# youngers2006/Dreamer

Hardware: AMD Instinct MI355X
Metric: imagined latent-steps/sec (B×H) at 64×64 CarRacing, 1/2/4/8 MI355X (higher is better)
Workload: dtype f32; 1 GPU; Dreamer.train_Agent() with AC_epochs=1 (replay sample + warm start S/2 + H-step imagination + actor-critic update), B=256/GPU S=64 H=15 64x64x3, precision=fp32 (north-star batch per GPU); global_batch=256, seq_len=64, horizon=15, parallelism=dp1, precision=fp32

## Files before the change

### dreamer_amd/csrc/conv_split.hip

```cpp
#include "conv.h"

#include <algorithm>
#include <climits>
#include <type_traits>

namespace {
typedef unsigned short u16;
typedef __bf16 bf16x8 __attribute__((ext_vector_type(8)));
typedef unsigned u32x4 __attribute__((ext_vector_type(4)));
typedef unsigned u32x2 __attribute__((ext_vector_type(2)));

__device__ __forceinline__ f32x4 mfma_b16(u32x4 a, u32x4 b, f32x4 c) {
  return __builtin_amdgcn_mfma_f32_16x16x32_bf16(__builtin_bit_cast(bf16x8, a), __builtin_bit_cast(bf16x8, b), c, 0, 0,
                                                  0);
}
__device__ __forceinline__ unsigned b16bits(__bf16 v) { return (unsigned)__builtin_bit_cast(u16, v); }
__device__ __forceinline__ void split3(float x, unsigned& h, unsigned& m, unsigned& l) {
  const __bf16 bh = (__bf16)x;
  const float r1 = x - (float)bh;
  const __bf16 bm = (__bf16)r1;
  const float r2 = r1 - (float)bm;
  h = b16bits(bh);
  m = b16bits(bm);
  l = b16bits((__bf16)r2);
}
__device__ __forceinline__ int swz(int row) { return (0x1320 >> (((row >> 2) & 3) * 4)) & 3; }
__device__ __forceinline__ u32x2 pack_bf16x4(f32x4 v) {
  typedef __bf16 bf16x4_t __attribute__((ext_vector_type(4)));
  const bf16x4_t b = {(__bf16)v[0], (__bf16)v[1], (__bf16)v[2], (__bf16)v[3]};
  return __builtin_bit_cast(u32x2, b);
}
__device__ __forceinline__ unsigned pack_bf16x2(float x0, float x1) { return b16bits((__bf16)x0) | (b16bits((__bf16)x1) << 16); }
}

template <int CIN>
__device__ __forceinline__ void conv_chunk(int c, int& tap, int& ci0, int& kc) {
  constexpr int CPT = CIN / 32;
  const int cc = c >> 4, t = c & 15;
  const int g = t >> 2, j = t & 3;
  const int ky = (g >> 1) + 2 * (j >> 1), kx = (g & 1) + 2 * (j & 1);
  tap = ky * 4 + kx;
  ci0 = 32 * cc;
  kc = tap * CPT + cc;
}

template <int BM, int BN, int CIN, bool OUT_NCHW, int PIPE, int EPI = CONV_EPI_FWD, int NT3 = 3, bool IO16 = (NT3 == 1)>
__global__ __launch_bounds__(BM * 2) void k_conv_split3(int n_frames, int ih, int iw, int cout,
                                                         const float* __restrict__ in, const u16* __restrict__ wr,
                                                         const float* __restrict__ bias, float* __restrict__ out,
                                                         float* __restrict__ pre) {
  static_assert(NT3 == 3 || (NT3 == 1 && (EPI == CONV_EPI_FWD || !IO16)), "conv_split3 terms");
  static_assert(!IO16 || NT3 == 1, "bf16 storage is the one-term form's");
  const u16* __restrict__ in16 = reinterpret_cast<const u16*>(in);
  u16* __restrict__ out16 = reinterpret_cast<u16*>(out);
  constexpr int NT = BM * 2;
  constexpr int K = CIN * 16;
  constexpr int NCH = K / 32;
  constexpr int WTN = BN / 2, FM = 4, FN = WTN / 16;
  constexpr int APT = BM * 8 / NT;
  constexpr int BU = NT3 * BN * 4;
  constexpr int BPT = (BU + NT - 1) / NT;
  static_assert(CIN % 32 == 0 && APT == 4 && FN >= 1, "conv_split3 tile");
  __shared__ __attribute__((aligned(16))) u32x4 As[2][NT3][BM][4];
  __shared__ __attribute__((aligned(16))) u32x4 Bs[2][NT3][BN][4];

  const int oh = ih / 2, ow = iw / 2, hw = oh * ow;
  const long long M = (long long)n_frames * hw;
  const int tiles_n = cout / BN;
  const long long tiles = ((M + BM - 1) / BM) * tiles_n;
  const int lt = dr_xcd_tile(blockIdx.x, (int)tiles);
  if (lt < 0) return;
  const long long m0 = (long long)(lt / tiles_n) * BM;
  const int n0 = (lt % tiles_n) * BN;
  const int tid = threadIdx.x, wave = tid >> 6, lane = tid & 63, r = lane & 15, q = lane >> 4;
  const int quad = tid & 7, prow = tid >> 3;

  int pb[APT];
  unsigned vm[APT];
#pragma unroll
  for (int i = 0; i < APT; ++i) {
    const long long m = m0 + prow + (NT / 8) * i;
    const int mm = (int)(m < M ? m : 0);
    const int f = mm / hw, p = mm - f * hw, oy = p / ow, ox = p - oy * ow;
    const int y0 = 2 * oy - 1, x0 = 2 * ox - 1;
    pb[i] = ((f * ih + y0) * iw + x0) * CIN;
    unsigned v = 0u;
#pragma unroll
    for (int t = 0; t < 4; ++t) {
      v |= (y0 + t >= 0 && y0 + t < ih) ? (1u << t) : 0u;
      v |= (x0 + t >= 0 && x0 + t < iw) ? (16u << t) : 0u;
    }
    vm[i] = m < M ? v : 0u;
  }

  f32x4 ra0[APT], ra1[APT];
  u32x2 rh0[APT], rh1[APT];
  u32x4 rb0[BPT], rb1[BPT];
  unsigned ok0 = 0, ok1 = 0;
  auto load = [&](int c, auto slot) __attribute__((always_inline)) {
    f32x4* ra = decltype(slot)::value == 0 ? ra0 : ra1;
    u32x2* rh = decltype(slot)::value == 0 ? rh0 : rh1;
    unsigned& okm = decltype(slot)::value == 0 ? ok0 : ok1;
    u32x4* rb = decltype(slot)::value == 0 ? rb0 : rb1;
    int tap, ci0, kc;
    conv_chunk<CIN>(c, tap, ci0, kc);
    const int ky = tap >> 2, kx = tap & 3;
    const int toff = (ky * iw + kx) * CIN + ci0 + 4 * quad;
    unsigned om = 0u;
#pragma unroll
    for (int i = 0; i < APT; ++i) {
      const bool ok = (vm[i] >> ky) & (vm[i] >> (4 + kx)) & 1u;
      if constexpr (IO16) rh[i] = *reinterpret_cast<const u32x2*>(in16 + (ok ? pb[i] + toff : 0));
      else ra[i] = *reinterpret_cast<const f32x4*>(in + (ok ? pb[i] + toff : 0));
      om |= ok ? (1u << i) : 0u;
    }
    okm = om;
#pragma unroll
    for (int j = 0; j < BPT; ++j) {
      const int e = tid + NT * j;
      if (BU % NT == 0 || e < BU) {
        const int pl = e / (BN * 4), rem = e - pl * BN * 4, row = rem >> 2, u = rem & 3;
        rb[j] = *reinterpret_cast<const u32x4*>(wr + (((long long)kc * 3 + pl) * cout + n0 + row) * 32 + 8 * u);
      }
    }
  };
  auto store = [&](auto slot, int buf) __attribute__((always_inline)) {
    const f32x4* ra = decltype(slot)::value == 0 ? ra0 : ra1;
    const u32x2* rh = decltype(slot)::value == 0 ? rh0 : rh1;
    const u32x4* rb = decltype(slot)::value == 0 ? rb0 : rb1;
    const unsigned okm = decltype(slot)::value == 0 ? ok0 : ok1;
#pragma unroll
    for (int i = 0; i < APT; ++i) {
      const int row = prow + (NT / 8) * i;
      const int unit = (quad >> 1) ^ swz(row), half = quad & 1;
      if constexpr (IO16) {
        reinterpret_cast<u32x2*>(&As[buf][0][row][unit])[half] = (okm >> i) & 1u ? rh[i] : (u32x2){0u, 0u};
      } else if constexpr (NT3 == 1) {
        const f32x4 v = (okm >> i) & 1u ? ra[i] : (f32x4){0.f, 0.f, 0.f, 0.f};
        reinterpret_cast<u32x2*>(&As[buf][0][row][unit])[half] = pack_bf16x4(v);
      } else {
        const f32x4 v = (okm >> i) & 1u ? ra[i] : (f32x4){0.f, 0.f, 0.f, 0.f};
        unsigned h0, m0_, l0, h1, m1, l1;
        split3_pair(v[0], v[1], h0, m0_, l0);
        split3_pair(v[2], v[3], h1, m1, l1);
        reinterpret_cast<u32x2*>(&As[buf][0][row][unit])[half] = (u32x2){h0, h1};
        reinterpret_cast<u32x2*>(&As[buf][1][row][unit])[half] = (u32x2){m0_, m1};
        reinterpret_cast<u32x2*>(&As[buf][2][row][unit])[half] = (u32x2){l0, l1};
      }
    }
#pragma unroll
    for (int j = 0; j < BPT; ++j) {
      const int e = tid + NT * j;
      if (BU % NT == 0 || e < BU) {
        const int pl = e / (BN * 4), rem = e - pl * BN * 4, row = rem >> 2, u = rem & 3;
        Bs[buf][pl][row][u ^ swz(row)] = rb[j];
      }
    }
  };

  const int wm0 = (wave >> 1) * 64, wn0 = (wave & 1) * WTN;
  const int fu = q ^ swz(r);
  f32x4 acc[FM][FN];
#pragma unroll
  for (int i = 0; i < FM; ++i)
#pragma unroll
    for (int j = 0; j < FN; ++j) acc[i][j] = (f32x4){0.f, 0.f, 0.f, 0.f};

  using S0 = std::integral_constant<int, 0>;
  using S1 = std::integral_constant<int, 1>;
  load(0, S0{});
  load(1, S1{});
  store(S0{}, 0);
  __syncthreads();
  auto step = [&](int c, auto slot) __attribute__((always_inline)) {
    constexpr int SL = decltype(slot)::value;
    using Next = std::integral_constant<int, 1 - SL>;
    const int buf = c & 1;
    load(min(c + PIPE, NCH - 1), slot);
    u32x4 a[NT3][FM], b[NT3][FN];
#pragma unroll
    for (int pl = 0; pl < NT3; ++pl) {
#pragma unroll
      for (int i = 0; i < FM; ++i) a[pl][i] = As[buf][pl][wm0 + 16 * i + r][fu];
#pragma unroll
      for (int j = 0; j < FN; ++j) b[pl][j] = Bs[buf][pl][wn0 + 16 * j + r][fu];
    }
#define DR_S3(PA, PB)                                                                                   \
  _Pragma("unroll") for (int i = 0; i < FM; ++i) _Pragma("unroll") for (int j = 0; j < FN; ++j) acc[i][j] = \
      OUT_NCHW ? mfma_b16(a[PA][i], b[PB][j], acc[i][j]) : mfma_b16(b[PB][j], a[PA][i], acc[i][j]);
    if constexpr (NT3 == 3) {
      DR_S3(2, 0)
      DR_S3(1, 1)
      DR_S3(0, 2)
      DR_S3(1, 0)
      DR_S3(0, 1)
    }
    DR_S3(0, 0)
#undef DR_S3
    if (c + 1 < NCH) store(Next{}, buf ^ 1);
    dr_lds_barrier();
  };
  static_assert(PIPE == 2 && NCH % 2 == 0, "conv_split3 ring");
  for (int c = 0; c < NCH; c += 2) {
    step(c, S0{});
    step(c + 1, S1{});
  }

#pragma unroll
  for (int i = 0; i < FM; ++i)
#pragma unroll
    for (int j = 0; j < FN; ++j) {
      if (OUT_NCHW) {
        const long long m = m0 + wm0 + 16 * i + 4 * q;
        const int co = n0 + wn0 + 16 * j + r;
        if (m >= M) continue;
        const float bv = bias[co];
        f32x4 v = acc[i][j] + bv;
        if constexpr (IO16) {
#pragma unroll
          for (int e = 0; e < 4; ++e) v[e] = dr_silu_fast(v[e]);
          const long long f = m / hw;
          *reinterpret_cast<u32x2*>(out16 + (f * cout + co) * hw + (m - f * hw)) = pack_bf16x4(v);
          continue;
        }
        if (pre) {
#pragma unroll
          for (int e = 0; e < 4; ++e) pre[(m + e) * cout + co] = v[e];
        }
#pragma unroll
        for (int e = 0; e < 4; ++e) v[e] = dr_silu_fast(v[e]);
        const long long f = m / hw;
        *reinterpret_cast<f32x4*>(out + (f * cout + co) * hw + (m - f * hw)) = v;
      } else {
        const long long m = m0 + wm0 + 16 * i + r;
        const int co = n0 + wn0 + 16 * j + 4 * q;
        if (m >= M) continue;
        f32x4 v;
        if (EPI == CONV_EPI_DSILU) {
          const f32x4 pv = *reinterpret_cast<const f32x4*>(pre + m * cout + co);
#pragma unroll
          for (int e = 0; e < 4; ++e) v[e] = acc[i][j][e] * dr_dsilu_fast(pv[e]);
        } else {
          const f32x4 bv = *reinterpret_cast<const f32x4*>(bias + co);
#pragma unroll
          for (int e = 0; e < 4; ++e) v[e] = acc[i][j][e] + bv[e];
          if (pre) *reinterpret_cast<f32x4*>(pre + m * cout + co) = v;
#pragma unroll
          for (int e = 0; e < 4; ++e) v[e] = dr_silu_fast(v[e]);
        }
        if constexpr (IO16) {
          *reinterpret_cast<u32x2*>(out16 + m * cout + co) = pack_bf16x4(v);
          continue;
        }
        *reinterpret_cast<f32x4*>(out + m * cout + co) = v;
      }
    }
}

__device__ __forceinline__ void conv_repack_split3_elem(int i, int cout, int cin, const float* __restrict__ w,
                                                        u16* __restrict__ wr) {
  const int co = i / (16 * cin), k = i - co * 16 * cin;
  const int tap = k / cin, ci = k - tap * cin;
  unsigned h, m, l;
  split3(w[((long long)co * cin + ci) * 16 + tap], h, m, l);
  const long long base = ((long long)(k >> 5) * 3 * cout + co) * 32 + (k & 31), plane = (long long)cout * 32;
  wr[base] = (u16)h;
  wr[base + plane] = (u16)m;
  wr[base + 2 * plane] = (u16)l;
}
__global__ void k_conv_repack_split3(int cout, int cin, const float* __restrict__ w, u16* __restrict__ wr) {
  const int i = blockIdx.x * blockDim.x + threadIdx.x;
  if (i >= cout * 16 * cin) return;
  conv_repack_split3_elem(i, cout, cin, w, wr);
}

int op_conv_repack_split3(int cout, int cin, const float* w, void* wr, hipStream_t s) {
  const int total = cout * 16 * cin;
  hipLaunchKernelGGL(k_conv_repack_split3, dim3((total + 255) / 256), dim3(256), 0, s, cout, cin, w, (u16*)wr);
  return dr_check_launch("conv_repack_split3");
}

#define E12_R2 8
#define E12_R1 (2 * E12_R2 + 2)
#define E12_RI (2 * E12_R1 + 2)
#define E12_PS (E12_R1 * 32 + 1)
#define E12_LWI 66
static constexpr size_t e12_lds_bytes(int terms = 3) {
  return (size_t)terms * 4 * E12_PS * 16 + (size_t)E12_RI * E12_LWI * 8;
}

#define DR_E12S1_WAVES 4
#define DR_E12S1_OCC 2
template <int NW, int NTM = 3, bool O16 = (NTM == 1)>
__global__ __launch_bounds__(64 * NW, NTM == 1 ? DR_E12S1_OCC : 1) void k_enc12_split3(int n, int nb, dr_frames src, const u16* __restrict__ wr1,
                                                          const float* __restrict__ b1, const u16* __restrict__ wr2,
                                                          const float* __restrict__ b2, float* __restrict__ out,
                                                          float* __restrict__ pre0, float* __restrict__ a0,
                                                          float* __restrict__ pre1) {
  static_assert((NW == 4 || NW == 8) && (NTM == 1 || NTM == 3) && (!O16 || NTM == 1), "enc12 waves / terms");
  constexpr int NTH = 64 * NW, TAPS = NW == 8 ? 8 : 16;
  constexpr int R2 = E12_R2, R1 = E12_R1, RI = E12_RI, PS = E12_PS, LWI = E12_LWI;
  constexpr int OW1 = 32, OW2 = 16, W = 64, H = 64, C1 = 32, C2 = 64;
  extern __shared__ __attribute__((aligned(16))) u32x4 e12_smem[];
  u32x4* c1o = e12_smem;
  uint2* xin = reinterpret_cast<uint2*>(e12_smem + NTM * 4 * PS);
  u16* xs = reinterpret_cast<u16*>(xin);
  u16* c1h = reinterpret_cast<u16*>(c1o);
  const int tid = threadIdx.x, wave = tid >> 6, lane = tid & 63, r = lane & 15, q = lane >> 4;
  const int ntiles = 2 * n;
  int tile = blockIdx.x;
  if (tile >= ntiles) return;

  for (int i = tid; i < RI * LWI; i += NTH) xin[i] = make_uint2(0u, 0u);
  constexpr int W4 = W / 4, PERC = RI * W4, MAXI = (3 * PERC + NTH - 1) / NTH;
  const unsigned hw = (unsigned)(H * W);
  const float centre = src.raw255 ? 127.5f : 0.0f, scale = src.raw255 ? 1.0f / 255.0f : 1.0f;
  unsigned uv[MAXI];
  auto in_load = [&](int tl) __attribute__((always_inline)) {
    const int f = tl >> 1, iy0 = 2 * (2 * (tl & 1) * R2 - 1) - 1;
    const int b = f % nb, t = f / nb + src.t0;
    const unsigned char* fr8 = src.ring + ((src.starts[b] + t) % src.ring_cap) * 3 * (long long)hw;
#pragma unroll
    for (int k = 0; k < MAXI; ++k) {
      const int i = tid + NTH * k;
      const int c = i / PERC, rem = i - c * PERC, rr = rem / W4, x4 = rem - rr * W4;
      const int y = iy0 + rr;
      const bool ok = i < 3 * PERC && y >= 0 && y < H;
      uv[k] = *reinterpret_cast<const unsigned*>(fr8 + (ok ? (unsigned)c * hw + (unsigned)(y * W + 4 * x4) : 0u));
    }
  };
  auto in_store = [&](int tl) __attribute__((always_inline)) {
    const int iy0 = 2 * (2 * (tl & 1) * R2 - 1) - 1;
#pragma unroll
    for (int k = 0; k < MAXI; ++k) {
      const int i = tid + NTH * k;
      if (i >= 3 * PERC) continue;
      const int c = i / PERC, rem = i - c * PERC, rr = rem / W4, x4 = rem - rr * W4;
      const int y = iy0 + rr;
      const bool ok = y >= 0 && y < H;
#pragma unroll
      for (int e = 0; e < 4; ++e)
        xs[(rr * LWI + 4 * x4 + e + 1) * 4 + c] =
            ok ? b16bits((__bf16)((float)((uv[k] >> (8 * e)) & 255u) - centre)) : (u16)0;
    }
  };
  in_load(tile);
  __syncthreads();
  in_store(tile);
  __syncthreads();

  const int w4 = wave & 3, kh = wave >> 2, ph = w4 & 1, ch = w4 >> 1;
  const u16* wbase = wr2 + ((long long)(32 * ch + r)) * 32 + 8 * q;
  auto wld = [&](u32x4 (&wf)[NTM][2], int tap) __attribute__((always_inline)) {
#pragma unroll
    for (int pl = 0; pl < NTM; ++pl)
#pragma unroll
      for (int jj = 0; jj < 2; ++jj)
        wf[pl][jj] = *reinterpret_cast<const u32x4*>(wbase + ((long long)(tap * 3 + pl) * C2 + 16 * jj) * 32);
  };

  for (;;) {
    const int f = tile >> 1, y2_0 = (tile & 1) * R2, y1_0 = 2 * y2_0 - 1;
    const int next = tile + (int)gridDim.x;
    u32x4 wa1[NTM][2][2];
#pragma unroll
    for (int pl = 0; pl < NTM; ++pl)
#pragma unroll
      for (int s = 0; s < 2; ++s)
#pragma unroll
        for (int j = 0; j < 2; ++j)
          wa1[pl][s][j] = *reinterpret_cast<const u32x4*>(wr1 + ((long long)pl * C1 + 16 * j + r) * 64 + 32 * s + 8 * q);
    float bb1[2][4];
#pragma unroll
    for (int j = 0; j < 2; ++j)
#pragma unroll
      for (int e = 0; e < 4; ++e) bb1[j][e] = b1[16 * j + 4 * q + e];
    u32x4 wfa[NTM][2], wfb[NTM][2];
    wld(wfa, TAPS * kh);
    constexpr int F1 = R1 * OW1 / 16;
    for (int i = wave; i < F1; i += NW) {
      const int p0 = 16 * i, yl = p0 / OW1, x1 = p0 - yl * OW1 + r, p = p0 + r;
      const int y1 = y1_0 + yl;
      uint2 hv[2], mv[2], lv[2];
      if (y1 < 0 || y1 >= H / 2) {
#pragma unroll
        for (int j = 0; j < 2; ++j) hv[j] = mv[j] = lv[j] = make_uint2(0u, 0u);
      } else {
        f32x4 acc[2] = {(f32x4){0.f, 0.f, 0.f, 0.f}, (f32x4){0.f, 0.f, 0.f, 0.f}};
#pragma unroll
        for (int s = 0; s < 2; ++s) {
          const int t0 = 8 * s + 2 * q, ky = t0 >> 2, kx = t0 & 3;
          const u32x4 pb = *reinterpret_cast<const u32x4*>(&xin[(2 * yl + ky) * LWI + 2 * x1 + kx]);
#pragma unroll
          for (int j = 0; j < 2; ++j) {
#pragma unroll
            for (int pl = NTM - 1; pl >= 0; --pl) acc[j] = mfma_b16(wa1[pl][s][j], pb, acc[j]);
          }
        }
        const bool own = !O16 && pre0 && yl >= 1 && yl <= 2 * R2;
        const long long o1 = (((long long)f * (H / 2) + y1) * OW1 + x1) * C1;
#pragma unroll
        for (int j = 0; j < 2; ++j) {
          float v[4], pv[4];
#pragma unroll
          for (int e = 0; e < 4; ++e) {
            pv[e] = acc[j][e] * scale + bb1[j][e];
            v[e] = dr_silu_fast(pv[e]);
          }
          if (own) {
            *reinterpret_cast<f32x4*>(pre0 + o1 + 16 * j + 4 * q) = (f32x4){pv[0], pv[1], pv[2], pv[3]};
            *reinterpret_cast<f32x4*>(a0 + o1 + 16 * j + 4 * q) = (f32x4){v[0], v[1], v[2], v[3]};
          }
          if constexpr (NTM == 1) {
            const u32x2 pk = pack_bf16x4((f32x4){v[0], v[1], v[2], v[3]});
            hv[j] = make_uint2(pk[0], pk[1]);
          } else {
            split3_pair(v[0], v[1], hv[j].x, mv[j].x, lv[j].x);
            split3_pair(v[2], v[3], hv[j].y, mv[j].y, lv[j].y);
          }
        }
      }
#pragma unroll
      for (int j = 0; j < 2; ++j) {
        const int c8 = 2 * j + (q >> 1);
        const int o = (c8 * PS + p) * 8 + (q & 1) * 4;
        *reinterpret_cast<uint2*>(c1h + o) = hv[j];
        if constexpr (NTM == 3) {
          *reinterpret_cast<uint2*>(c1h + 4 * PS * 8 + o) = mv[j];
          *reinterpret_cast<uint2*>(c1h + 2 * 4 * PS * 8 + o) = lv[j];
        }
      }
    }
    __syncthreads();
    if (next < ntiles) in_load(next);

    f32x4 acc[4][2];
#pragma unroll
    for (int i = 0; i < 4; ++i)
#pragma unroll
      for (int jj = 0; jj < 2; ++jj) acc[i][jj] = (f32x4){0.f, 0.f, 0.f, 0.f};
    auto tap_step = [&](int tap, u32x4 (&wf)[NTM][2], u32x4 (&wn)[NTM][2]) __attribute__((always_inline)) {
      wld(wn, tap + 1 < TAPS * (kh + 1) ? tap + 1 : tap);
      const int ky = tap >> 2, kx = tap & 3;
      const int x1 = 2 * r - 1 + kx;
      const bool xok = x1 >= 0 && x1 < OW1;
      u32x4 pf[NTM][4];
#pragma unroll
      for (int i = 0; i < 4; ++i) {
        const int yl = 2 * (4 * ph + i) + ky;
        const int u = q * PS + yl * OW1 + (xok ? x1 : 0);
#pragma unroll
        for (int pl = 0; pl < NTM; ++pl) {
          const u32x4 v = c1o[pl * 4 * PS + u];
          pf[pl][i] = xok ? v : (u32x4){0u, 0u, 0u, 0u};
        }
      }
#define E12_S3(PW, PA)                       \
  _Pragma("unroll") for (int i = 0; i < 4; ++i) _Pragma("unroll") for (int jj = 0; jj < 2; ++jj) acc[i][jj] = \
      mfma_b16(wf[PW][jj], pf[PA][i], acc[i][jj]);
      if constexpr (NTM == 3) {
        E12_S3(2, 0)
        E12_S3(1, 1)
        E12_S3(0, 2)
        E12_S3(1, 0)
        E12_S3(0, 1)
      }
      E12_S3(0, 0)
#undef E12_S3
    };
#pragma unroll 1
    for (int tap = TAPS * kh; tap < TAPS * (kh + 1); ++tap) {
      tap_step(tap, wfa, wfb);
#pragma unroll
      for (int pl = 0; pl < NTM; ++pl)
#pragma unroll
        for (int jj = 0; jj < 2; ++jj) wfa[pl][jj] = wfb[pl][jj];
    }
    if (NW == 8) {
      f32x4* red = reinterpret_cast<f32x4*>(e12_smem);
      __syncthreads();
      if (kh == 1) {
#pragma unroll
        for (int i = 0; i < 4; ++i)
#pragma unroll
          for (int jj = 0; jj < 2; ++jj) red[(w4 * 8 + i * 2 + jj) * 64 + lane] = acc[i][jj];
      }
      __syncthreads();
      if (kh == 0) {
#pragma unroll
        for (int i = 0; i < 4; ++i)
#pragma unroll
          for (int jj = 0; jj < 2; ++jj) acc[i][jj] += red[(w4 * 8 + i * 2 + jj) * 64 + lane];
      }
    }
#pragma unroll
    for (int i = 0; i < 4; ++i) {
      if (kh) break;
      float* o = out + (((long long)f * OW2 + y2_0 + 4 * ph + i) * OW2 + r) * C2;
#pragma unroll
      for (int jj = 0; jj < 2; ++jj) {
        const int co = 32 * ch + 16 * jj + 4 * q;
        const f32x4 bv = *reinterpret_cast<const f32x4*>(b2 + co);
        f32x4 v;
        const f32x4 pv = acc[i][jj] + bv;
#pragma unroll
        for (int e = 0; e < 4; ++e) v[e] = dr_silu_fast(pv[e]);
        if constexpr (O16) {
          *reinterpret_cast<u32x2*>(reinterpret_cast<u16*>(out) + (o - out) + co) = pack_bf16x4(v);
          continue;
        }
        *reinterpret_cast<f32x4*>(o + co) = v;
        if (pre1) *reinterpret_cast<f32x4*>(pre1 + (o - out) + co) = pv;
      }
    }
    if (next >= ntiles) break;
    in_store(next);
    __syncthreads();
    tile = next;
  }
}

__device__ __forceinline__ void conv1_repack_split3_elem(int i, int cout, const float* __restrict__ w,
                                                         u16* __restrict__ wr) {
  const int co = i >> 6, k = i & 63, tap = k >> 2, c = k & 3;
  unsigned h, m, l;
  split3(c < 3 ? w[((long long)co * 3 + c) * 16 + tap] : 0.f, h, m, l);
  wr[i] = (u16)h;
  wr[cout * 64 + i] = (u16)m;
  wr[2 * cout * 64 + i] = (u16)l;
}
__global__ void k_conv1_repack_split3(int cout, const float* __restrict__ w, u16* __restrict__ wr) {
  const int i = blockIdx.x * blockDim.x + threadIdx.x;
  if (i >= cout * 64) return;
  conv1_repack_split3_elem(i, cout, w, wr);
}

bool op_enc12_split3_ok(int n, int h, int w, int c1, int c2, const dr_frames* src) {
  return c1 == 32 && c2 == 64 && h == 64 && w == 64 && src->ring && src->starts && src->ring_cap > 0 && n > 0 &&
         (long long)n * 2 < (1LL << 31);
}

int op_enc12_split3(int n, int nb, int h, int w, int c1, int c2, const dr_frames* src, const float* w1,
                    const float* b1, const float* w2, const float* b2, void* wr1, void* wr2, float* out,
                    hipStream_t s, int prepacked) {
  return op_enc12_split3_ex(n, nb, h, w, c1, c2, src, w1, b1, w2, b2, wr1, wr2, out, nullptr, nullptr, nullptr, s, 3,
                            prepacked);
}

int op_enc12_split3_ex(int n, int nb, int h, int w, int c1, int c2, const dr_frames* src, const float* w1,
                       const float* b1, const float* w2, const float* b2, void* wr1, void* wr2, float* out,
                       float* pre0, float* a0, float* pre1, hipStream_t s, int terms, int prepacked) {
  if ((pre0 != nullptr) != (a0 != nullptr) || ((uintptr_t)pre0 | (uintptr_t)a0 | (uintptr_t)pre1) & 15 ||
      (terms != 1 && terms != 3))
    return DR_E_INVALID;
  if (!op_enc12_split3_ok(n, h, w, c1, c2, src)) return DR_E_INVALID;
  static const bool raised = [] {
    (void)hipFuncSetAttribute((const void*)k_enc12_split3<4>, hipFuncAttributeMaxDynamicSharedMemorySize,
                              (int)e12_lds_bytes());
    (void)hipFuncSetAttribute((const void*)k_enc12_split3<8>, hipFuncAttributeMaxDynamicSharedMemorySize,
                              (int)e12_lds_bytes());
    return true;
  }();
  (void)raised;
  if (!prepacked) {
    hipLaunchKernelGGL(k_conv1_repack_split3, dim3((c1 * 64 + 255) / 256), dim3(256), 0, s, c1, w1, (u16*)wr1);
    DR_TRY(dr_check_launch("conv1_repack_split3"));
    DR_TRY(op_conv_repack_split3(c2, c1, w2, wr2, s));
  }
  if (terms == 1) {
    static int slots1[64];
    int dev = 0;
    DR_TRY_HIP(hipGetDevice(&dev));
    if (dev < 0 || dev >= 64) return DR_E_INVALID;
    auto kf = k_enc12_split3<DR_E12S1_WAVES, 1, false>;
    if (slots1[dev] == 0) {
      (void)hipFuncSetAttribute((const void*)kf, hipFuncAttributeMaxDynamicSharedMemorySize, (int)e12_lds_bytes(1));
      int cus = 0, per = 0;
      DR_TRY_HIP(hipDeviceGetAttribute(&cus, hipDeviceAttributeMultiprocessorCount, dev));
      DR_TRY_HIP(hipOccupancyMaxActiveBlocksPerMultiprocessor(&per, kf, 64 * DR_E12S1_WAVES, e12_lds_bytes(1)));
      slots1[dev] = std::max(1, per) * std::max(1, cus);
    }
    const int grid = std::min(n * 2, slots1[dev]);
    hipLaunchKernelGGL(kf, dim3((unsigned)grid), dim3(64 * DR_E12S1_WAVES), e12_lds_bytes(1), s, n, nb, *src,
                       (const u16*)wr1, b1, (const u16*)wr2, b2, out, pre0, a0, pre1);
    return dr_check_launch("enc12_split3 (one term)");
  }
  static int cus[64];
  int dev = 0;
  DR_TRY_HIP(hipGetDevice(&dev));
  if (dev < 0 || dev >= 64) return DR_E_INVALID;
  if (cus[dev] == 0) DR_TRY_HIP(hipDeviceGetAttribute(&cus[dev], hipDeviceAttributeMultiprocessorCount, dev));
  const int grid = std::min(n * 2, std::max(1, cus[dev]));
  hipLaunchKernelGGL(k_enc12_split3<8>, dim3((unsigned)grid), dim3(512), e12_lds_bytes(), s, n, nb, *src,
                     (const u16*)wr1, b1, (const u16*)wr2, b2, out, pre0, a0, pre1);
  return dr_check_launch("enc12_split3");
}

int op_enc12_s1_bf16(int n, int nb, int h, int w, int c1, int c2, const dr_frames* src, const float* w1,
                     const float* b1, const float* w2, const float* b2, void* wr1, void* wr2, void* out,
                     hipStream_t s, int prepacked) {
  if (!op_enc12_split3_ok(n, h, w, c1, c2, src) || ((uintptr_t)out & 15)) return DR_E_INVALID;
  static int slots[64];
  int dev = 0;
  DR_TRY_HIP(hipGetDevice(&dev));
  if (dev < 0 || dev >= 64) return DR_E_INVALID;
  if (slots[dev] == 0) {
    (void)hipFuncSetAttribute((const void*)k_enc12_split3<DR_E12S1_WAVES, 1>, hipFuncAttributeMaxDynamicSharedMemorySize,
                              (int)e12_lds_bytes(1));
    int cus = 0, per = 0;
    DR_TRY_HIP(hipDeviceGetAttribute(&cus, hipDeviceAttributeMultiprocessorCount, dev));
    DR_TRY_HIP(hipOccupancyMaxActiveBlocksPerMultiprocessor(&per, k_enc12_split3<DR_E12S1_WAVES, 1>,
                                                            64 * DR_E12S1_WAVES, e12_lds_bytes(1)));
    slots[dev] = std::max(1, per) * std::max(1, cus);
  }
  if (!prepacked) {
    hipLaunchKernelGGL(k_conv1_repack_split3, dim3((c1 * 64 + 255) / 256), dim3(256), 0, s, c1, w1, (u16*)wr1);
    DR_TRY(dr_check_launch("conv1_repack_split3"));
    DR_TRY(op_conv_repack_split3(c2, c1, w2, wr2, s));
  }
  const int grid = std::min(n * 2, slots[dev]);
  hipLaunchKernelGGL((k_enc12_split3<DR_E12S1_WAVES, 1>), dim3((unsigned)grid), dim3(64 * DR_E12S1_WAVES),
                     e12_lds_bytes(1), s, n, nb, *src,
                     (const u16*)wr1, b1, (const u16*)wr2, b2, (float*)out, nullptr, nullptr, nullptr);
  return dr_check_launch("enc12_s1_bf16");
}

template <int BM, int BN, int CIN, bool NCHW, int PIPE, int EPI = CONV_EPI_FWD, int TERMS = 3>
static int launch_s3(int n, int ih, int iw, int cout, const float* in, const void* wr, const float* bias, float* out,
                     float* pre, hipStream_t s) {
  const long long M = (long long)n * (ih / 2) * (iw / 2);
  const long long tiles = ((M + BM - 1) / BM) * (cout / BN);
  if (tiles >= (1LL << 30)) {
    dr_set_error("conv_split3: too many tiles");
    return DR_E_INVALID;
  }
  hipLaunchKernelGGL((k_conv_split3<BM, BN, CIN, NCHW, PIPE, EPI, TERMS, false>), dim3((unsigned)dr_xcd_grid((int)tiles)),
                     dim3(BM * 2), 0, s, n, ih, iw, cout, in, (const u16*)wr, bias, out, pre);
  return dr_check_launch("conv_split3");
}

bool op_conv_split3_supported(int n, int cin, int ih, int iw, int cout) {
  const bool cin_ok = cin == 32 || cin == 64 || cin == 128 || cin == 256;
  return cin_ok && cout % 64 == 0 && ih % 2 == 0 && iw % 2 == 0 && ((ih / 2) * (iw / 2)) % 4 == 0 &&
         (long long)n * ih * iw * cin < (1LL << 31) - (1LL << 20);
}

int op_conv_split3_ex(int n, int cin, int ih, int iw, int cout, const float* in, const void* wr, const float* bias,
                      float* out, int out_nchw, float* pre, int epi, hipStream_t s, int terms) {
  if (!op_conv_split3_supported(n, cin, ih, iw, cout) || (terms != 1 && terms != 3)) {
    dr_set_error("conv_split3: unsupported shape (cin=%d ih=%d iw=%d cout=%d)", cin, ih, iw, cout);
    return DR_E_INVALID;
  }
  if (epi == CONV_EPI_DSILU && (out_nchw || !pre)) {
    dr_set_error("conv_split3: the SiLU-backward epilogue needs NHWC output and a pre-activation tensor");
    return DR_E_INVALID;
  }
  if (terms == 3 && (epi == CONV_EPI_FWD ? bias != nullptr : pre != nullptr) && op_conv_glds_s3_supported(n, cin, ih, iw, cout) &&
      !(((uintptr_t)in | (uintptr_t)wr | (uintptr_t)out | (uintptr_t)bias | (uintptr_t)pre) & 15))
    return op_conv_glds_s3(n, cin, ih, iw, cout, in, wr, bias, out, out_nchw, pre, epi, s);
#define DR_S3E(BN, C, NCHW, T)                                                                                         \
  (epi == CONV_EPI_DSILU ? launch_s3<256, BN, C, NCHW, 2, CONV_EPI_DSILU, T>(n, ih, iw, cout, in, wr, bias, out, pre, s) \
                         : launch_s3<256, BN, C, NCHW, 2, CONV_EPI_FWD, T>(n, ih, iw, cout, in, wr, bias, out, pre, s))
#define DR_S3L(C, T)                                                                                                 \
  if (cin == C) {                                                                                                    \
    if (cout % 128 == 0)                                                                                             \
      return out_nchw ? launch_s3<256, 128, C, true, 2, CONV_EPI_FWD, T>(n, ih, iw, cout, in, wr, bias, out, pre, s) \
                      : DR_S3E(128, C, false, T);                                                                    \
    return out_nchw ? launch_s3<256, 64, C, true, 2, CONV_EPI_FWD, T>(n, ih, iw, cout, in, wr, bias, out, pre, s)    \
                    : DR_S3E(64, C, false, T);                                                                       \
  }
  if (terms == 1) {
    DR_S3L(32, 1)
    DR_S3L(64, 1)
    DR_S3L(128, 1)
    DR_S3L(256, 1)
  } else {
    DR_S3L(32, 3)
    DR_S3L(64, 3)
    DR_S3L(128, 3)
    DR_S3L(256, 3)
  }
#undef DR_S3L
#undef DR_S3E
  return DR_E_INVALID;
}

int op_conv_split3(int n, int cin, int ih, int iw, int cout, const float* in, const void* wr, const float* bias,
                   float* out, int out_nchw, hipStream_t s) {
  return op_conv_split3_ex(n, cin, ih, iw, cout, in, wr, bias, out, out_nchw, nullptr, CONV_EPI_FWD, s);
}

template <int BN, int C, bool NCHW>
static int launch_s1(int n, int ih, int iw, int cout, const void* in, const void* wr, const float* bias, void* out,
                     hipStream_t s) {
  const long long M = (long long)n * (ih / 2) * (iw / 2);
  const long long tiles = ((M + 255) / 256) * (cout / BN);
  if (tiles >= (1LL << 30)) {
    dr_set_error("conv_s1_bf16: too many tiles");
    return DR_E_INVALID;
  }
  hipLaunchKernelGGL((k_conv_split3<256, BN, C, NCHW, 2, CONV_EPI_FWD, 1>), dim3((unsigned)dr_xcd_grid((int)tiles)),
                     dim3(512), 0, s, n, ih, iw, cout, (const float*)in, (const u16*)wr, bias, (float*)out, nullptr);
  return dr_check_launch("conv_s1_bf16");
}

int op_conv_s1_bf16(int n, int cin, int ih, int iw, int cout, const void* in, const void* wr, const float* bias,
                    void* out, int out_nchw, hipStream_t s) {
  if (!op_conv_split3_supported(n, cin, ih, iw, cout) || (((uintptr_t)in | (uintptr_t)out | (uintptr_t)bias) & 15)) {
    dr_set_error("conv_s1_bf16: unsupported shape (cin=%d ih=%d iw=%d cout=%d)", cin, ih, iw, cout);
    return DR_E_INVALID;
  }
  if (op_conv_glds_bf16_supported(n, cin, ih, iw, cout))
    return op_conv_glds_bf16(n, cin, ih, iw, cout, in, wr, bias, out, out_nchw, s);
#define DR_S1L(C)                                                                              \
  if (cin == C) {                                                                              \
    if (cout % 128 == 0)                                                                       \
      return out_nchw ? launch_s1<128, C, true>(n, ih, iw, cout, in, wr, bias, out, s)         \
                      : launch_s1<128, C, false>(n, ih, iw, cout, in, wr, bias, out, s);       \
    return out_nchw ? launch_s1<64, C, true>(n, ih, iw, cout, in, wr, bias, out, s)            \
                    : launch_s1<64, C, false>(n, ih, iw, cout, in, wr, bias, out, s);          \
  }
  DR_S1L(32)
  DR_S1L(64)
  DR_S1L(128)
  DR_S1L(256)
#undef DR_S1L
  return DR_E_INVALID;
}

template <int BM, int BN, int CIN, int EPI, int TERMS = 3>
__global__ __launch_bounds__(BM * 2) void k_convT_split3(ConvTArgs a, const u16* __restrict__ wr) {
  constexpr int NT = BM * 2;
  constexpr int K = CIN * 4;
  constexpr int NCH = K / 32;
  constexpr int WTN = BN / 2, FM = 4, FN = WTN / 16;
  constexpr int APT = BM * 8 / NT;
  constexpr int BU = TERMS * BN * 4;
  constexpr int BPT = (BU + NT - 1) / NT;
  static_assert(CIN % 32 == 0 && APT == 4 && FN >= 1 && NCH % 2 == 0 && (TERMS == 1 || TERMS == 3),
                "convT_split3 tile");
  __shared__ __attribute__((aligned(16))) u32x4 As[2][TERMS][BM][4];
  __shared__ __attribute__((aligned(16))) u32x4 Bs[2][TERMS][BN][4];

  const int h = a.h, w = a.w, hw = h * w, cout = a.cout;
  const long long M = (long long)a.n * hw;
  const int tiles_n = cout / BN;
  const long long tiles_m = (M + BM - 1) / BM;
  const int lt = dr_xcd_tile(blockIdx.x, (int)(4 * tiles_m * tiles_n));
  if (lt < 0) return;
  const int cls = lt & 3;
  const long long rem = lt >> 2;
  const long long m0 = (rem / tiles_n) * BM;
  const int n0 = (int)(rem % tiles_n) * BN;
  const int py = cls >> 1, px = cls & 1;
  const int tid = threadIdx.x, wave = tid >> 6, lane = tid & 63, r = lane & 15, q = lane >> 4;
  const int quad = tid & 7, prow = tid >> 3;
  const float* __restrict__ in = a.in;
  const u16* __restrict__ wc = wr + (long long)cls * NCH * 3 * cout * 32;

  int pb[APT];
  unsigned vm[APT];
#pragma unroll
  for (int i = 0; i < APT; ++i) {
    const long long m = m0 + prow + (NT / 8) * i;
    const int mm = (int)(m < M ? m : 0);
    const int f = mm / hw, p = mm - f * hw, y = p / w, x = p - y * w;
    pb[i] = ((f * h + y) * w + x) * CIN;
    unsigned v = 0u;
#pragma unroll
    for (int t = 0; t < 4; ++t) {
      const int iy = y + py - (t >> 1), ix = x + px - (t & 1);
      v |= (iy >= 0 && iy < h && ix >= 0 && ix < w) ? (1u << t) : 0u;
    }
    vm[i] = m < M ? v : 0u;
  }

  f32x4 ra0[APT], ra1[APT];
  u32x4 rb0[BPT], rb1[BPT];
  unsigned ok0 = 0, ok1 = 0;
  auto load = [&](int c, auto slot) __attribute__((always_inline)) {
    f32x4* ra = decltype(slot)::value == 0 ? ra0 : ra1;
    unsigned& okm = decltype(slot)::value == 0 ? ok0 : ok1;
    u32x4* rb = decltype(slot)::value == 0 ? rb0 : rb1;
    const int tap = (32 * c) / CIN, ci0 = 32 * c - tap * CIN;
    const int toff = ((py - (tap >> 1)) * w + (px - (tap & 1))) * CIN + ci0 + 4 * quad;
    unsigned om = 0u;
#pragma unroll
    for (int i = 0; i < APT; ++i) {
      const bool ok = (vm[i] >> tap) & 1u;
      ra[i] = *reinterpret_cast<const f32x4*>(in + (ok ? pb[i] + toff : 0));
      om |= ok ? (1u << i) : 0u;
    }
    okm = om;
#pragma unroll
    for (int j = 0; j < BPT; ++j) {
      const int e = tid + NT * j;
      if (BU % NT == 0 || e < BU) {
        const int pl = e / (BN * 4), rm = e - pl * BN * 4, row = rm >> 2, u = rm & 3;
        rb[j] = *reinterpret_cast<const u32x4*>(wc + (((long long)c * 3 + pl) * cout + n0 + row) * 32 + 8 * u);
      }
    }
  };
  auto store = [&](auto slot, int buf) __attribute__((always_inline)) {
    const f32x4* ra = decltype(slot)::value == 0 ? ra0 : ra1;
    const u32x4* rb = decltype(slot)::value == 0 ? rb0 : rb1;
    const unsigned okm = decltype(slot)::value == 0 ? ok0 : ok1;
#pragma unroll
    for (int i = 0; i < APT; ++i) {
      const int row = prow + (NT / 8) * i;
      const f32x4 v = (okm >> i) & 1u ? ra[i] : (f32x4){0.f, 0.f, 0.f, 0.f};
      const int unit = (quad >> 1) ^ swz(row), half = quad & 1;
      if constexpr (TERMS == 1) {
        reinterpret_cast<u32x2*>(&As[buf][0][row][unit])[half] = pack_bf16x4(v);
      } else {
        unsigned h0, m0_, l0, h1, m1, l1;
        split3_pair(v[0], v[1], h0, m0_, l0);
        split3_pair(v[2], v[3], h1, m1, l1);
        reinterpret_cast<u32x2*>(&As[buf][0][row][unit])[half] = (u32x2){h0, h1};
        reinterpret_cast<u32x2*>(&As[buf][1][row][unit])[half] = (u32x2){m0_, m1};
        reinterpret_cast<u32x2*>(&As[buf][2][row][unit])[half] = (u32x2){l0, l1};
      }
    }
#pragma unroll
    for (int j = 0; j < BPT; ++j) {
      const int e = tid + NT * j;
      if (BU % NT == 0 || e < BU) {
        const int pl = e / (BN * 4), rm = e - pl * BN * 4, row = rm >> 2, u = rm & 3;
        Bs[buf][pl][row][u ^ swz(row)] = rb[j];
      }
    }
  };

  const int wm0 = (wave >> 1) * 64, wn0 = (wave & 1) * WTN;
  const int fu = q ^ swz(r);
  f32x4 acc[FM][FN];
#pragma unroll
  for (int i = 0; i < FM; ++i)
#pragma unroll
    for (int j = 0; j < FN; ++j) acc[i][j] = (f32x4){0.f, 0.f, 0.f, 0.f};

  using S0 = std::integral_constant<int, 0>;
  using S1 = std::integral_constant<int, 1>;
  load(0, S0{});
  load(1, S1{});
  store(S0{}, 0);
  __syncthreads();
  auto step = [&](int c, auto slot) __attribute__((always_inline)) {
    constexpr int SL = decltype(slot)::value;
    using Next = std::integral_constant<int, 1 - SL>;
    const int buf = c & 1;
    load(min(c + 2, NCH - 1), slot);
    u32x4 av[TERMS][FM], bv[TERMS][FN];
#pragma unroll
    for (int pl = 0; pl < TERMS; ++pl) {
#pragma unroll
      for (int i = 0; i < FM; ++i) av[pl][i] = As[buf][pl][wm0 + 16 * i + r][fu];
#pragma unroll
      for (int j = 0; j < FN; ++j) bv[pl][j] = Bs[buf][pl][wn0 + 16 * j + r][fu];
    }
#define DR_T3(PA, PB)                                                                                   \
  _Pragma("unroll") for (int i = 0; i < FM; ++i) _Pragma("unroll") for (int j = 0; j < FN; ++j) acc[i][j] = \
      mfma_b16(bv[PB][j], av[PA][i], acc[i][j]);
    if constexpr (TERMS == 3) {
      DR_T3(2, 0)
      DR_T3(1, 1)
      DR_T3(0, 2)
      DR_T3(1, 0)
      DR_T3(0, 1)
    }
    DR_T3(0, 0)
#undef DR_T3
    if (c + 1 < NCH) store(Next{}, buf ^ 1);
    dr_lds_barrier();
  };
  for (int c = 0; c < NCH; c += 2) {
    step(c, S0{});
    step(c + 1, S1{});
  }

  const int OW = 2 * w, OH = 2 * h;
#pragma unroll
  for (int i = 0; i < FM; ++i) {
    const long long m = m0 + wm0 + 16 * i + r;
    if (m >= M) continue;
    const int f = (int)(m / hw), p = (int)(m - (long long)f * hw), y = p / w, x = p - y * w;
    const long long opix = ((long long)f * OH + 2 * y + py) * OW + 2 * x + px;
#pragma unroll
    for (int j = 0; j < FN; ++j) {
      const int co = n0 + wn0 + 16 * j + 4 * q;
      f32x4 v = acc[i][j];
      if (EPI == CT_EPI_BIAS) {
        v += *reinterpret_cast<const f32x4*>(a.bias + co);
        f32x4 sv = v;
        if (a.out2 || a.silu_out) {
#pragma unroll
          for (int e = 0; e < 4; ++e) sv[e] = dr_silu_fast(v[e]);
        }
// ... 1294 lines not shown
```

Baseline: 611,700 imagined latent-steps/s.

## Add restructured 8-wave enc12 split3 kernel with padded LDS and double-buffered taps

Adds a new fused conv1+conv2 encoder kernel for the 3-term split path. It pads the conv1 output rows in LDS so taps need no x bounds checks, and hoists the conv1 weight loads out of the tile loop. It double-buffers both weight and patch fragments across taps, and splits the cross-wave reduction so both halves of the waves write outputs. The next tile's input is staged before the output stores. Optional timestamp instrumentation is added behind a compile flag, and the old kernel is kept only under that flag.

Result: faster. 618,200 imagined latent-steps/s, median of 6 (+1.1%).

```diff
diff --git a/dreamer_amd/csrc/conv_split.hip b/dreamer_amd/csrc/conv_split.hip
--- a/dreamer_amd/csrc/conv_split.hip
+++ b/dreamer_amd/csrc/conv_split.hip
@@ -288,6 +288,27 @@
 static constexpr size_t e12_lds_bytes(int terms = 3) {
   return (size_t)terms * 4 * E12_PS * 16 + (size_t)E12_RI * E12_LWI * 8;
 }
+
+#define E12_TS_WGS 4
+#define E12_TS_TILES 4
+#define E12_TS_MARKS 8
+#ifdef DR_E12_TS
+__device__ long long dr_e12_ts_buf[E12_TS_WGS * E12_TS_TILES * 2 * E12_TS_MARKS];
+#define E12_TS(tile, k)                                                                                        \
+  do {                                                                                                         \
+    const int it_ = ((tile) - (int)blockIdx.x) / (int)gridDim.x;                                               \
+    if ((threadIdx.x & 255) == 0 && blockIdx.x < E12_TS_WGS && it_ < E12_TS_TILES)                             \
+      dr_e12_ts_buf[((blockIdx.x * E12_TS_TILES + it_) * 2 + (threadIdx.x >> 8)) * E12_TS_MARKS + (k)] =       \
+          (long long)wall_clock64();                                                                           \
+  } while (0)
+extern "C" int dr_e12_ts_read(long long* host) {
+  return hipMemcpyFromSymbol(host, HIP_SYMBOL(dr_e12_ts_buf), sizeof(dr_e12_ts_buf)) == hipSuccess ? 0 : -1;
+}
+#else
+#define E12_TS(tile, k) \
+  do {                  \
+  } while (0)
+#endif
 
 #define DR_E12S1_WAVES 4
 #define DR_E12S1_OCC 2
@@ -362,6 +383,7 @@
   for (;;) {
     const int f = tile >> 1, y2_0 = (tile & 1) * R2, y1_0 = 2 * y2_0 - 1;
     const int next = tile + (int)gridDim.x;
+    E12_TS(tile, 0);
     u32x4 wa1[NTM][2][2];
 #pragma unroll
     for (int pl = 0; pl < NTM; ++pl)
@@ -431,7 +453,9 @@
         }
       }
     }
+    E12_TS(tile, 1);
     __syncthreads();
+    E12_TS(tile, 2);
     if (next < ntiles) in_load(next);
 
     f32x4 acc[4][2];
@@ -476,6 +500,7 @@
 #pragma unroll
         for (int jj = 0; jj < 2; ++jj) wfa[pl][jj] = wfb[pl][jj];
     }
+    E12_TS(tile, 3);
     if (NW == 8) {
       f32x4* red = reinterpret_cast<f32x4*>(e12_smem);
       __syncthreads();
@@ -493,6 +518,7 @@
           for (int jj = 0; jj < 2; ++jj) acc[i][jj] += red[(w4 * 8 + i * 2 + jj) * 64 + lane];
       }
     }
+    E12_TS(tile, 4);
 #pragma unroll
     for (int i = 0; i < 4; ++i) {
       if (kh) break;
@@ -513,9 +539,263 @@
         if (pre1) *reinterpret_cast<f32x4*>(pre1 + (o - out) + co) = pv;
       }
     }
+    E12_TS(tile, 5);
     if (next >= ntiles) break;
     in_store(next);
     __syncthreads();
+    E12_TS(tile, 6);
+    tile = next;
+  }
+}
+
+#define E12X_OW 34
+#define E12X_PS (E12_R1 * E12X_OW + 1)
+#define E12X_XCH (8 * 4 * 64 * 16)
+static constexpr size_t e12x_lds_bytes() { return (size_t)3 * 4 * E12X_PS * 16 + E12X_XCH; }
+static_assert(E12X_XCH >= E12_RI * E12_LWI * 8 && e12x_lds_bytes() <= 160 * 1024, "enc12 LDS");
+
+__global__ __launch_bounds__(512, 1) void k_enc12_split3_x8(int n, int nb, dr_frames src, const u16* __restrict__ wr1,
+                                                            const float* __restrict__ b1, const u16* __restrict__ wr2,
+                                                            const float* __restrict__ b2, float* __restrict__ out,
+                                                            float* __restrict__ pre0, float* __restrict__ a0,
+                                                            float* __restrict__ pre1) {
+  constexpr int NTH = 512, TAPS = 8;
+  constexpr int R2 = E12_R2, R1 = E12_R1, RI = E12_RI, PS = E12X_PS, OWP = E12X_OW, LWI = E12_LWI;
+  constexpr int OW1 = 32, OW2 = 16, W = 64, H = 64, C1 = 32, C2 = 64;
+  extern __shared__ __attribute__((aligned(16))) u32x4 e12_smem[];
+  u32x4* c1o = e12_smem;
+  uint2* xin = reinterpret_cast<uint2*>(e12_smem + 3 * 4 * PS);
+  f32x4* xch = reinterpret_cast<f32x4*>(e12_smem + 3 * 4 * PS);
+  u16* c1h = reinterpret_cast<u16*>(c1o);
+  const int tid = threadIdx.x, wave = __builtin_amdgcn_readfirstlane(tid >> 6), lane = tid & 63, r = lane & 15,
+            q = lane >> 4;
+  const int ntiles = 2 * n;
+  int tile = blockIdx.x;
+  if (tile >= ntiles) return;
+
+  for (int i = tid; i < 3 * 4 * R1 * 2; i += NTH) {
+    const int pc = i / (2 * R1), rem = i - pc * 2 * R1;
+    c1o[pc * PS + (rem >> 1) * OWP + (rem & 1) * (OWP - 1)] = (u32x4){0u, 0u, 0u, 0u};
+  }
+  constexpr int NIT = RI * (W / 4), MAXI = (NIT + NTH - 1) / NTH;
+  const unsigned hw = (unsigned)(H * W);
+  const float centre = src.raw255 ? 127.5f : 0.0f, scale = src.raw255 ? 1.0f / 255.0f : 1.0f;
+  unsigned uv[MAXI][3];
+  auto in_load = [&](int tl) __attribute__((always_inline)) {
+    const int f = tl >> 1, iy0 = 2 * (2 * (tl & 1) * R2 - 1) - 1;
+    const int b = f % nb, t = f / nb + src.t0;
+    const unsigned char* fr8 = src.ring + ((src.starts[b] + t) % src.ring_cap) * 3 * (long long)hw;
+#pragma unroll
+    for (int k = 0; k < MAXI; ++k) {
+      const int i = tid + NTH * k, rr = i >> 4, x4 = i & 15, y = iy0 + rr;
+      const bool ok = i < NIT && y >= 0 && y < H;
+#pragma unroll
+      for (int c = 0; c < 3; ++c)
+        uv[k][c] = *reinterpret_cast<const unsigned*>(fr8 + (ok ? (unsigned)c * hw + (unsigned)(y * W + 4 * x4) : 0u));
+    }
+  };
+  auto in_store = [&](int tl) __attribute__((always_inline)) {
+    const int iy0 = 2 * (2 * (tl & 1) * R2 - 1) - 1;
+#pragma unroll
+    for (int k = 0; k < MAXI; ++k) {
+      const int i = tid + NTH * k, rr = i >> 4, x4 = i & 15, y = iy0 + rr;
+      if (i >= NIT) continue;
+      const bool ok = y >= 0 && y < H;
+#pragma unroll
+      for (int e = 0; e < 4; ++e) {
+        unsigned bb[3];
+#pragma unroll
+        for (int c = 0; c < 3; ++c) bb[c] = b16bits((__bf16)((float)((uv[k][c] >> (8 * e)) & 255u) - centre));
+        xin[rr * LWI + 4 * x4 + e + 1] = ok ? make_uint2(bb[0] | (bb[1] << 16), bb[2]) : make_uint2(0u, 0u);
+      }
+      if (x4 == 0) xin[rr * LWI] = make_uint2(0u, 0u);
+      if (x4 == W / 4 - 1) xin[rr * LWI + LWI - 1] = make_uint2(0u, 0u);
+    }
+  };
+  in_load(tile);
+  u32x4 wa1[3][2][2];
+  float bb1[2][4];
+#pragma unroll
+  for (int pl = 0; pl < 3; ++pl)
+#pragma unroll
+    for (int s = 0; s < 2; ++s)
+#pragma unroll
+      for (int j = 0; j < 2; ++j)
+        wa1[pl][s][j] = *reinterpret_cast<const u32x4*>(wr1 + ((long long)pl * C1 + 16 * j + r) * 64 + 32 * s + 8 * q);
+#pragma unroll
+  for (int j = 0; j < 2; ++j)
+#pragma unroll
+    for (int e = 0; e < 4; ++e) bb1[j][e] = b1[16 * j + 4 * q + e];
+  in_store(tile);
+  __syncthreads();
+
+  const int w4 = wave & 3, kh = wave >> 2, ph = w4 & 1, ch = w4 >> 1;
+  const u16* wbase = wr2 + ((long long)(32 * ch + r)) * 32 + 8 * q;
+  auto wld = [&](u32x4 (&wf)[3][2], int tap) __attribute__((always_inline)) {
+#pragma unroll
+    for (int pl = 0; pl < 3; ++pl)
+#pragma unroll
+      for (int jj = 0; jj < 2; ++jj)
+        wf[pl][jj] = *reinterpret_cast<const u32x4*>(wbase + ((long long)(tap * 3 + pl) * C2 + 16 * jj) * 32);
+  };
+  auto pld = [&](u32x4 (&pf)[3][4], int tap) __attribute__((always_inline)) {
+    const int ky = tap >> 2, kx = tap & 3;
+#pragma unroll
+    for (int i = 0; i < 4; ++i) {
+      const int u = q * PS + (2 * (4 * ph + i) + ky) * OWP + 2 * r + kx;
+#pragma unroll
+      for (int pl = 0; pl < 3; ++pl) pf[pl][i] = c1o[pl * 4 * PS + u];
+    }
+  };
+
+  for (;;) {
+    const int f = tile >> 1, y2_0 = (tile & 1) * R2, y1_0 = 2 * y2_0 - 1;
+    const int next = tile + (int)gridDim.x;
+    E12_TS(tile, 0);
+    u32x4 wfa[3][2], wfb[3][2];
+    wld(wfa, TAPS * kh);
+    auto c1_block = [&](int i, auto JM) __attribute__((always_inline)) {
+      constexpr int jm = decltype(JM)::value;
+      const int yl = i >> 1, x1 = 16 * (i & 1) + r, y1 = y1_0 + yl;
+      uint2 hv[2], mv[2], lv[2];
+      if (y1 < 0 || y1 >= H / 2) {
+#pragma unroll
+        for (int j = 0; j < 2; ++j) hv[j] = mv[j] = lv[j] = make_uint2(0u, 0u);
+      } else {
+        f32x4 acc[2] = {(f32x4){0.f, 0.f, 0.f, 0.f}, (f32x4){0.f, 0.f, 0.f, 0.f}};
+#pragma unroll
+        for (int s = 0; s < 2; ++s) {
+          const int t0 = 8 * s + 2 * q, ky = t0 >> 2, kx = t0 & 3;
+          const u32x4 pb = *reinterpret_cast<const u32x4*>(&xin[(2 * yl + ky) * LWI + 2 * x1 + kx]);
+#pragma unroll
+          for (int j = 0; j < 2; ++j) {
+            if (!((jm >> j) & 1)) continue;
+#pragma unroll
+            for (int pl = 2; pl >= 0; --pl) acc[j] = mfma_b16(wa1[pl][s][j], pb, acc[j]);
+          }
+        }
+        const bool own = pre0 && yl >= 1 && yl <= 2 * R2;
+        const long long o1 = (((long long)f * (H / 2) + y1) * OW1 + x1) * C1;
+#pragma unroll
+        for (int j = 0; j < 2; ++j) {
+          if (!((jm >> j) & 1)) continue;
+          float v[4], pv[4];
+#pragma unroll
+          for (int e = 0; e < 4; ++e) {
+            pv[e] = acc[j][e] * scale + bb1[j][e];
+            v[e] = dr_silu_fast(pv[e]);
+          }
+          if (own) {
+            *reinterpret_cast<f32x4*>(pre0 + o1 + 16 * j + 4 * q) = (f32x4){pv[0], pv[1], pv[2], pv[3]};
+            *reinterpret_cast<f32x4*>(a0 + o1 + 16 * j + 4 * q) = (f32x4){v[0], v[1], v[2], v[3]};
+          }
+          split3_pair(v[0], v[1], hv[j].x, mv[j].x, lv[j].x);
+          split3_pair(v[2], v[3], hv[j].y, mv[j].y, lv[j].y);
+        }
+      }
+#pragma unroll
+      for (int j = 0; j < 2; ++j) {
+        if (!((jm >> j) & 1)) continue;
+        const int c8 = 2 * j + (q >> 1);
+        const int o = (c8 * PS + yl * OWP + x1 + 1) * 8 + (q & 1) * 4;
+        *reinterpret_cast<uint2*>(c1h + o) = hv[j];
+        *reinterpret_cast<uint2*>(c1h + 4 * PS * 8 + o) = mv[j];
+        *reinterpret_cast<uint2*>(c1h + 2 * 4 * PS * 8 + o) = lv[j];
+      }
+    };
+    constexpr int F1 = R1 * OW1 / 16;
+    static_assert(F1 == 36, "conv1 block split");
+    for (int i = wave; i < 32; i += 8) c1_block(i, std::integral_constant<int, 3>());
+    if (wave & 1)
+      c1_block(32 + (wave >> 1), std::integral_constant<int, 2>());
+    else
+      c1_block(32 + (wave >> 1), std::integral_constant<int, 1>());
+    E12_TS(tile, 1);
+    dr_lds_barrier();
+    E12_TS(tile, 2);
+    if (next < ntiles) in_load(next);
+
+    f32x4 acc[4][2];
+#pragma unroll
+    for (int i = 0; i < 4; ++i)
+#pragma unroll
+      for (int jj = 0; jj < 2; ++jj) acc[i][jj] = (f32x4){0.f, 0.f, 0.f, 0.f};
+    auto tap_mm = [&](u32x4 (&wf)[3][2], u32x4 (&pf)[3][4]) __attribute__((always_inline)) {
+#define E12_S3(PW, PA)                       \
+  _Pragma("unroll") for (int i = 0; i < 4; ++i) _Pragma("unroll") for (int jj = 0; jj < 2; ++jj) acc[i][jj] = \
+      mfma_b16(wf[PW][jj], pf[PA][i], acc[i][jj]);
+      E12_S3(2, 0)
+      E12_S3(1, 1)
+      E12_S3(0, 2)
+      E12_S3(1, 0)
+      E12_S3(0, 1)
+      E12_S3(0, 0)
+#undef E12_S3
+    };
+    {
+      const int tap0 = TAPS * kh, last = tap0 + TAPS - 1;
+      u32x4 pfa[3][4], pfb[3][4];
+      pld(pfa, tap0);
+#pragma unroll 1
+      for (int tap = tap0; tap < last; tap += 2) {
+        wld(wfb, tap + 1);
+        pld(pfb, tap + 1);
+        tap_mm(wfa, pfa);
+        const int tn = tap + 2 < last ? tap + 2 : last;
+        wld(wfa, tn);
+        pld(pfa, tn);
+        tap_mm(wfb, pfb);
+      }
+    }
+    E12_TS(tile, 3);
+    f32x4 fin[2][2];
+    if (kh) {
+#pragma unroll
+      for (int il = 0; il < 2; ++il)
+#pragma unroll
+        for (int jj = 0; jj < 2; ++jj) xch[(wave * 4 + il * 2 + jj) * 64 + lane] = acc[il][jj];
+    } else {
+#pragma unroll
+      for (int il = 0; il < 2; ++il)
+#pragma unroll
+        for (int jj = 0; jj < 2; ++jj) xch[(wave * 4 + il * 2 + jj) * 64 + lane] = acc[2 + il][jj];
+    }
+    dr_lds_barrier();
+    if (kh) {
+#pragma unroll
+      for (int il = 0; il < 2; ++il)
+#pragma unroll
+        for (int jj = 0; jj < 2; ++jj) fin[il][jj] = xch[((wave - 4) * 4 + il * 2 + jj) * 64 + lane] + acc[2 + il][jj];
+    } else {
+#pragma unroll
+      for (int il = 0; il < 2; ++il)
+#pragma unroll
+        for (int jj = 0; jj < 2; ++jj) fin[il][jj] = acc[il][jj] + xch[((wave + 4) * 4 + il * 2 + jj) * 64 + lane];
+    }
+    E12_TS(tile, 4);
+    if (next < ntiles) {
+      dr_lds_barrier();
+      in_store(next);
+      dr_lds_barrier();
+    }
+    E12_TS(tile, 5);
+#pragma unroll
+    for (int il = 0; il < 2; ++il) {
+      float* o = out + (((long long)f * OW2 + y2_0 + 4 * ph + 2 * kh + il) * OW2 + r) * C2;
+#pragma unroll
+      for (int jj = 0; jj < 2; ++jj) {
+        const int co = 32 * ch + 16 * jj + 4 * q;
+        const f32x4 bv = *reinterpret_cast<const f32x4*>(b2 + co);
+        f32x4 v;
+        const f32x4 pv = fin[il][jj] + bv;
+#pragma unroll
+        for (int e = 0; e < 4; ++e) v[e] = dr_silu_fast(pv[e]);
+        *reinterpret_cast<f32x4*>(o + co) = v;
+        if (pre1) *reinterpret_cast<f32x4*>(pre1 + (o - out) + co) = pv;
+      }
+    }
+    E12_TS(tile, 6);
+    if (next >= ntiles) break;
     tile = next;
   }
 }
@@ -557,8 +837,12 @@
   static const bool raised = [] {
     (void)hipFuncSetAttribute((const void*)k_enc12_split3<4>, hipFuncAttributeMaxDynamicSharedMemorySize,
                               (int)e12_lds_bytes());
+    (void)hipFuncSetAttribute((const void*)k_enc12_split3_x8, hipFuncAttributeMaxDynamicSharedMemorySize,
+                              (int)e12x_lds_bytes());
+#if defined(DR_E12_TS) && DR_E12_TS == 2
     (void)hipFuncSetAttribute((const void*)k_enc12_split3<8>, hipFuncAttributeMaxDynamicSharedMemorySize,
                               (int)e12_lds_bytes());
+#endif
     return true;
   }();
   (void)raised;
@@ -591,8 +875,13 @@
   if (dev < 0 || dev >= 64) return DR_E_INVALID;
   if (cus[dev] == 0) DR_TRY_HIP(hipDeviceGetAttribute(&cus[dev], hipDeviceAttributeMultiprocessorCount, dev));
   const int grid = std::min(n * 2, std::max(1, cus[dev]));
+#if defined(DR_E12_TS) && DR_E12_TS == 2
   hipLaunchKernelGGL(k_enc12_split3<8>, dim3((unsigned)grid), dim3(512), e12_lds_bytes(), s, n, nb, *src,
                      (const u16*)wr1, b1, (const u16*)wr2, b2, out, pre0, a0, pre1);
+#else
+  hipLaunchKernelGGL(k_enc12_split3_x8, dim3((unsigned)grid), dim3(512), e12x_lds_bytes(), s, n, nb, *src,
+                     (const u16*)wr1, b1, (const u16*)wr2, b2, out, pre0, a0, pre1);
+#endif
   return dr_check_launch("enc12_split3");
 }
 
```
